# jannerm/ddpo

Measured on AMD Instinct MI355X. Metric: sampled images/sec (512^2, 50 DDIM steps), higher is better.
Workload: dtype f32 (f16mx: f16 MFMA + MX-fp8 cross terms on the long-reduction conv/GEMM layers, bf16x3-split MFMA elsewhere); 1 GPU; BASELINE configs[1]: compressed-animals geometry, sd15 U-Net+VAE (random init), 512x512, 50 DDIM steps, CFG 5.0, eta 1.0, sample_batch_size 8/GPU, VAE decode included; parallelism=dp1, global_batch=8

## Files before the change

ddpo_amd/csrc/attention_bf16.hip:

```cpp
#include "common.h"
#include <cstdlib>


typedef __bf16 bf16x8 __attribute__((ext_vector_type(8)));
typedef _Float16 f16x8 __attribute__((ext_vector_type(8)));
typedef _Float16 f16x2 __attribute__((ext_vector_type(2)));
typedef float f32x16 __attribute__((ext_vector_type(16)));

typedef __bf16 bf16x2 __attribute__((ext_vector_type(2)));
__device__ __forceinline__ uint32_t cvt_pk_bf16_a(float lo, float hi) {
  const bf16x2 v = {(__bf16)lo, (__bf16)hi};
  return __builtin_bit_cast(uint32_t, v);
}
__device__ __forceinline__ uint32_t cvt_pk_f16_a(float lo, float hi) {
  const f16x2 v = {(_Float16)lo, (_Float16)hi};
  return __builtin_bit_cast(uint32_t, v);
}
__device__ __forceinline__ void split2(float a, float b, uint32_t& hi, uint32_t& lo) {
  hi = cvt_pk_bf16_a(a, b);
  lo = cvt_pk_bf16_a(a - __uint_as_float(hi << 16), b - __uint_as_float(hi & 0xFFFF0000u));
}
__device__ __forceinline__ void split2h(float a, float b, uint32_t& hi, uint32_t& lo) {
  const float lim = 65504.f;
  a = fminf(fmaxf(a, -lim), lim);
// ... 87 lines not shown
                                                     bool& grew) {
  float mx = sacc[0][0];
#pragma unroll
  for (int j = 0; j < 2; ++j)
#pragma unroll
    for (int r = 0; r < 16; ++r) mx = fmaxf(mx, sacc[j][r]);
  mx = fmaxf(mx, __shfl_xor(mx, 32, 64));
  const float m_new = fmaxf(m_run, mx);
  alpha = __builtin_amdgcn_exp2f(m_run - m_new);
  grew = m_new > m_run;
  m_run = m_new;
  float ls = 0.f;
#pragma unroll
  for (int j = 0; j < 2; ++j) {
#pragma unroll
    for (int half = 0; half < 2; ++half) {
      uint32_t hi[4], lo[4];
#pragma unroll
      for (int e = 0; e < 4; ++e) {
        const float p0 = __builtin_amdgcn_exp2f(sacc[j][8 * half + 2 * e] - m_new);
        const float p1 = __builtin_amdgcn_exp2f(sacc[j][8 * half + 2 * e + 1] - m_new);
        ls += p0 + p1;
        split2(p0, p1, hi[e], lo[e]);
      }
      ph[2 * j + half] = __builtin_bit_cast(bf16x8, make_uint4(hi[0], hi[1], hi[2], hi[3]));
      pl[2 * j + half] = __builtin_bit_cast(bf16x8, make_uint4(lo[0], lo[1], lo[2], lo[3]));
    }
  }
  l_run = l_run * alpha + ls;
}

template <int NDT, int LDVT, int QB = 1>
__device__ __forceinline__ void attn_pv_tile_x3(const char* Vhi, const char* Vlo, int li, int h, const bf16x8 (*ph)[4], const bf16x8 (*pl)[4],
                                                f32x16 (*oacc)[NDT]) {
#pragma unroll
  for (int u = 0; u < 4; ++u) {
#pragma unroll
    for (int n = 0; n < NDT; ++n) {
      const int off = ((32 * n + li) * LDVT + 16 * u + 4 * h) * 2;
      const uint2 a0 = *reinterpret_cast<const uint2*>(Vhi + off), a1 = *reinterpret_cast<const uint2*>(Vhi + off + 16);
      const uint2 c0 = *reinterpret_cast<const uint2*>(Vlo + off), c1 = *reinterpret_cast<const uint2*>(Vlo + off + 16);
      const bf16x8 vh = __builtin_bit_cast(bf16x8, make_uint4(a0.x, a0.y, a1.x, a1.y));
      const bf16x8 vl = __builtin_bit_cast(bf16x8, make_uint4(c0.x, c0.y, c1.x, c1.y));
#pragma unroll
      for (int qb = 0; qb < QB; ++qb) {
        oacc[qb][n] = MFMA32(vl, ph[qb][u], oacc[qb][n]);
        oacc[qb][n] = MFMA32(vh, pl[qb][u], oacc[qb][n]);
        oacc[qb][n] = MFMA32(vh, ph[qb][u], oacc[qb][n]);
      }
    }
  }
}

template <bool F16P, bool ONES, int NDT, int LDVT>
__device__ __forceinline__ void attn_tile_tail(const f32x16 (&sacc)[2], float& m_run, float& l_run, f32x16 (&oacc)[NDT], const char* Vhi, const char* Vlo,
                                               int li, int h) {
  float alpha;
  bool grew;
  if constexpr (F16P) {
    f16x8 ph[4];
    attn_softmax_tile<ONES>(sacc, m_run, l_run, ph, alpha, grew);
    if (__any(grew)) {
#pragma unroll
      for (int n = 0; n < NDT; ++n)
#pragma unroll
        for (int r = 0; r < 16; ++r) oacc[n][r] *= alpha;
    }
    attn_pv_tile<NDT, LDVT>(Vhi, Vlo, li, h, &ph, &oacc);
  } else {
    bf16x8 ph[4], pl[4];
    attn_softmax_tile_x3(sacc, m_run, l_run, ph, pl, alpha, grew);
    if (__any(grew)) {
#pragma unroll
      for (int n = 0; n < NDT; ++n)
#pragma unroll
        for (int r = 0; r < 16; ++r) oacc[n][r] *= alpha;
    }
    attn_pv_tile_x3<NDT, LDVT>(Vhi, Vlo, li, h, &ph, &pl, &oacc);
  }
}

struct AttnOut {
  float* o;
  uint16_t* hi;
  uint16_t* lo;
  int ld;
  int64_t rows;
};
template <int D, int NDT>
__device__ __forceinline__ void attn_store_o(const AttnOut out, int64_t row, int col0, const f32x16 (&oacc)[NDT], float inv, int h) {
#pragma unroll
  for (int n = 0; n < NDT; ++n) {
#pragma unroll
    for (int g = 0; g < 4; ++g) {
      const int dc = 32 * n + 8 * g + 4 * h;
      if (dc >= D) continue;
      const float v0 = oacc[n][4 * g] * inv, v1 = oacc[n][4 * g + 1] * inv, v2 = oacc[n][4 * g + 2] * inv, v3 = oacc[n][4 * g + 3] * inv;
      if (out.hi) {
        uint32_t h0, l0, h1, l1;
        split2(v0, v1, h0, l0);
        split2(v2, v3, h1, l1);
        const int64_t off = plane_off(row, col0 + dc, out.ld, out.rows);
        *reinterpret_cast<uint2*>(out.hi + off) = make_uint2(h0, h1);
        *reinterpret_cast<uint2*>(out.lo + off) = make_uint2(l0, l1);
      } else {
        *reinterpret_cast<float4*>(out.o + row * out.ld + col0 + dc) = make_float4(v0, v1, v2, v3);
      }
    }
  }
}


template <int D, int DKP, int DVP, bool F16P>
__global__ void __launch_bounds__(256) attn_fwd_bf16_kernel(const float* __restrict__ q, int ldq, const float* __restrict__ k, int ldk,
                                                            const float* __restrict__ v, int ldv, const AttnOut out,
                                                            float* __restrict__ lse, int heads, int Nq, int Nk, float scale_log2e) {
  constexpr int KT = 64;
  constexpr int LDK = DKP + 8;
  constexpr int LDVT = KT + 4;
  constexpr int NKS = DKP / 16;
  constexpr int NDT = DVP / 32;
  constexpr bool ONES = F16P && DVP > D;
  constexpr int K_BYTES = KT * LDK * 2, VT_BYTES = DVP * LDVT * 2;
  __shared__ __attribute__((aligned(16))) char smem[2 * K_BYTES + 2 * VT_BYTES];
  char* Khi = smem; char* Klo = smem + K_BYTES;
  char* Vhi = smem + 2 * K_BYTES; char* Vlo = Vhi + VT_BYTES;

  const int t = threadIdx.x, lane = t & 63, wid = t >> 6;
  const int li = lane & 31, h = lane >> 5;
  const int bh = blockIdx.y, b = bh / heads, hd = bh - b * heads;
  const int q0 = blockIdx.x * 128 + wid * 32;
  const int qrow = min(q0 + li, Nq - 1);

  bf16x8 qh[NKS], ql[NKS];
  {
    const float* qp = q + ((int64_t)b * Nq + qrow) * ldq + hd * D;
#pragma unroll
    for (int s = 0; s < NKS; ++s) {
      uint32_t hi[4], lo[4];
#pragma unroll
      for (int e = 0; e < 4; ++e) {
        const int dk = 16 * s + 8 * h + 2 * e;
        const float a = dk < D ? qp[dk] * scale_log2e : 0.f;
        const float c = dk + 1 < D ? qp[dk + 1] * scale_log2e : 0.f;
        split2(a, c, hi[e], lo[e]);
      }
      qh[s] = __builtin_bit_cast(bf16x8, make_uint4(hi[0], hi[1], hi[2], hi[3]));
      ql[s] = __builtin_bit_cast(bf16x8, make_uint4(lo[0], lo[1], lo[2], lo[3]));
    }
  }
  for (int i = t; i < (2 * K_BYTES + 2 * VT_BYTES) / 16; i += 256) reinterpret_cast<uint4*>(smem)[i] = make_uint4(0u, 0u, 0u, 0u);
  if constexpr (ONES) {
    __syncthreads();
    if (t < KT) reinterpret_cast<uint16_t*>(Vhi)[D * LDVT + t] = (uint16_t)ATTN_F16_ONE;
  }

  f32x16 oacc[NDT];
#pragma unroll
  for (int n = 0; n < NDT; ++n)
#pragma unroll
    for (int r = 0; r < 16; ++r) oacc[n][r] = 0.f;
  float m_run = -INFINITY, l_run = 0.f;
  const float* kb = k + (int64_t)b * Nk * ldk + hd * D;
  const float* vb = v + (int64_t)b * Nk * ldv + hd * D;

  for (int kt0 = 0; kt0 < Nk; kt0 += KT) {
    __syncthreads();
    for (int i = t; i < KT * (D / 4); i += 256) {
      const int key = i / (D / 4), c4 = i - key * (D / 4);
      float4 kv = make_float4(0.f, 0.f, 0.f, 0.f), vv = kv;
      if (kt0 + key < Nk) {
        kv = *reinterpret_cast<const float4*>(kb + (int64_t)(kt0 + key) * ldk + c4 * 4);
        vv = *reinterpret_cast<const float4*>(vb + (int64_t)(kt0 + key) * ldv + c4 * 4);
      }
      uint32_t h0, l0, h1, l1;
      split2(kv.x, kv.y, h0, l0);
      split2(kv.z, kv.w, h1, l1);
      *reinterpret_cast<uint2*>(Khi + (key * LDK + c4 * 4) * 2) = make_uint2(h0, h1);
      *reinterpret_cast<uint2*>(Klo + (key * LDK + c4 * 4) * 2) = make_uint2(l0, l1);
      if (F16P) { split2h(vv.x, vv.y, h0, l0); split2h(vv.z, vv.w, h1, l1); }
      else { split2(vv.x, vv.y, h0, l0); split2(vv.z, vv.w, h1, l1); }
      uint16_t* vh = reinterpret_cast<uint16_t*>(Vhi);
      uint16_t* vl = reinterpret_cast<uint16_t*>(Vlo);
      const int d0 = c4 * 4;
      vh[(d0 + 0) * LDVT + key] = (uint16_t)(h0 & 0xFFFFu); vh[(d0 + 1) * LDVT + key] = (uint16_t)(h0 >> 16);
      vh[(d0 + 2) * LDVT + key] = (uint16_t)(h1 & 0xFFFFu); vh[(d0 + 3) * LDVT + key] = (uint16_t)(h1 >> 16);
      vl[(d0 + 0) * LDVT + key] = (uint16_t)(l0 & 0xFFFFu); vl[(d0 + 1) * LDVT + key] = (uint16_t)(l0 >> 16);
      vl[(d0 + 2) * LDVT + key] = (uint16_t)(l1 & 0xFFFFu); vl[(d0 + 3) * LDVT + key] = (uint16_t)(l1 >> 16);
    }
    __syncthreads();

    f32x16 sacc[2];
#pragma unroll
    for (int j = 0; j < 2; ++j)
#pragma unroll
      for (int r = 0; r < 16; ++r) sacc[j][r] = 0.f;
#pragma unroll
    for (int s = 0; s < NKS; ++s) {
#pragma unroll
      for (int j = 0; j < 2; ++j) {
        const int off = ((j * 32 + li) * LDK + 16 * s + 8 * h) * 2;
        const bf16x8 kh = *reinterpret_cast<const bf16x8*>(Khi + off);
        const bf16x8 kl = *reinterpret_cast<const bf16x8*>(Klo + off);
        sacc[j] = MFMA32(kl, qh[s], sacc[j]);
        sacc[j] = MFMA32(kh, ql[s], sacc[j]);
        sacc[j] = MFMA32(kh, qh[s], sacc[j]);
      }
    }
    if (kt0 + KT > Nk) {
#pragma unroll
      for (int j = 0; j < 2; ++j)
#pragma unroll
        for (int r = 0; r < 16; ++r)
          if (kt0 + 32 * j + (r & 3) + 8 * (r >> 2) + 4 * h >= Nk) sacc[j][r] = -INFINITY;
    }
    attn_tile_tail<F16P, ONES, NDT, LDVT>(sacc, m_run, l_run, oacc, Vhi, Vlo, li, h);
  }

  const float l_tot = attn_row_sum<D, NDT, ONES>(oacc, l_run, li);
  const float inv = 1.0f / l_tot;
  if (lse && h == 0 && q0 + li < Nq) lse[(int64_t)bh * Nq + q0 + li] = m_run + log2f(l_tot) - (F16P ? ATTN_P_SHIFT : 0.f);
  if (q0 + li < Nq) attn_store_o<D, NDT>(out, (int64_t)b * Nq + q0 + li, hd * D, oacc, inv, h);
}

template <int D, int DKP, int DVP>
struct AttnImg {
  static constexpr int KT = 64, LDK = DKP + 8, LDVT = KT + 4;
  static constexpr int K_BYTES = KT * LDK * 2, VT_BYTES = DVP * LDVT * 2;
  static constexpr int BYTES = 2 * K_BYTES + 2 * VT_BYTES;
  static constexpr int CHUNKS = BYTES / 16;
};

template <int D, int DKP, int DVP, bool F16P>
__global__ void __launch_bounds__(256) attn_pack_kv_kernel(const float* __restrict__ k, int ldk, const float* __restrict__ v, int ldv,
                                                           uint4* __restrict__ img, int heads, int Nk, int ntiles) {
  using I = AttnImg<D, DKP, DVP>;
  __shared__ __attribute__((aligned(16))) char smem[I::BYTES];
  char* Khi = smem; char* Klo = smem + I::K_BYTES;
  char* Vhi = smem + 2 * I::K_BYTES; char* Vlo = Vhi + I::VT_BYTES;
  const int t = threadIdx.x;
  const int tile = blockIdx.x, bh = blockIdx.y, b = bh / heads, hd = bh - b * heads;
  const int kt0 = tile * I::KT;
  for (int i = t; i < I::CHUNKS; i += 256) reinterpret_cast<uint4*>(smem)[i] = make_uint4(0u, 0u, 0u, 0u);
  __syncthreads();
  if (F16P && DVP > D && t < I::KT) reinterpret_cast<uint16_t*>(Vhi)[D * I::LDVT + t] = (uint16_t)ATTN_F16_ONE;
  const float* kb = k + (int64_t)b * Nk * ldk + hd * D;
  const float* vb = v + (int64_t)b * Nk * ldv + hd * D;
  for (int i = t; i < I::KT * (D / 4); i += 256) {
    const int key = i / (D / 4), c4 = i - key * (D / 4);
    if (kt0 + key >= Nk) continue;
    const float4 kv = *reinterpret_cast<const float4*>(kb + (int64_t)(kt0 + key) * ldk + c4 * 4);
    const float4 vv = *reinterpret_cast<const float4*>(vb + (int64_t)(kt0 + key) * ldv + c4 * 4);
    uint32_t h0, l0, h1, l1;
    split2(kv.x, kv.y, h0, l0);
    split2(kv.z, kv.w, h1, l1);
    *reinterpret_cast<uint2*>(Khi + (key * I::LDK + c4 * 4) * 2) = make_uint2(h0, h1);
    *reinterpret_cast<uint2*>(Klo + (key * I::LDK + c4 * 4) * 2) = make_uint2(l0, l1);
    if (F16P) { split2h(vv.x, vv.y, h0, l0); split2h(vv.z, vv.w, h1, l1); }
    else { split2(vv.x, vv.y, h0, l0); split2(vv.z, vv.w, h1, l1); }
    uint16_t* vh = reinterpret_cast<uint16_t*>(Vhi);
    uint16_t* vl = reinterpret_cast<uint16_t*>(Vlo);
    const int d0 = c4 * 4;
    vh[(d0 + 0) * I::LDVT + key] = (uint16_t)(h0 & 0xFFFFu); vh[(d0 + 1) * I::LDVT + key] = (uint16_t)(h0 >> 16);
    vh[(d0 + 2) * I::LDVT + key] = (uint16_t)(h1 & 0xFFFFu); vh[(d0 + 3) * I::LDVT + key] = (uint16_t)(h1 >> 16);
    vl[(d0 + 0) * I::LDVT + key] = (uint16_t)(l0 & 0xFFFFu); vl[(d0 + 1) * I::LDVT + key] = (uint16_t)(l0 >> 16);
    vl[(d0 + 2) * I::LDVT + key] = (uint16_t)(l1 & 0xFFFFu); vl[(d0 + 3) * I::LDVT + key] = (uint16_t)(l1 >> 16);
  }
  __syncthreads();
  uint4* dst = img + ((int64_t)bh * ntiles + tile) * I::CHUNKS;
  for (int i = t; i < I::CHUNKS; i += 256) dst[i] = reinterpret_cast<const uint4*>(smem)[i];
}

template <int D, int DKP, int DVP, bool F16P>
__global__ void __launch_bounds__(256, (DVP <= 32 ? 4 : (DKP <= 48 ? 3 : 2))) attn_fwd_bf16_pk_kernel(const float* __restrict__ q, int ldq, const uint4* __restrict__ img,
                                                               const AttnOut out, float* __restrict__ lse, int heads,
                                                               int Nq, int Nk, int ntiles, float scale_log2e) {
  using I = AttnImg<D, DKP, DVP>;
  constexpr int KT = I::KT, LDK = I::LDK, LDVT = I::LDVT;
  constexpr int NKS = DKP / 16, NDT = DVP / 32;
  constexpr bool ONES = F16P && DVP > D;
  constexpr int NCH = (I::CHUNKS + 255) / 256;
  __shared__ __attribute__((aligned(16))) char smem[I::BYTES];
  const char* Khi = smem; const char* Klo = smem + I::K_BYTES;
  const char* Vhi = smem + 2 * I::K_BYTES; const char* Vlo = Vhi + I::VT_BYTES;

  const int t = threadIdx.x, lane = t & 63, wid = t >> 6;
  const int li = lane & 31, h = lane >> 5;
  const int bh = blockIdx.y, b = bh / heads, hd = bh - b * heads;
  const int q0 = blockIdx.x * 128 + wid * 32;
  const int qrow = min(q0 + li, Nq - 1);

  bf16x8 qh[NKS], ql[NKS];
  {
    const float* qp = q + ((int64_t)b * Nq + qrow) * ldq + hd * D;
#pragma unroll
    for (int s = 0; s < NKS; ++s) {
      uint32_t hi[4], lo[4];
#pragma unroll
      for (int e = 0; e < 4; ++e) {
        const int dk = 16 * s + 8 * h + 2 * e;
        const float a = dk < D ? qp[dk] * scale_log2e : 0.f;
        const float c = dk + 1 < D ? qp[dk + 1] * scale_log2e : 0.f;
        split2(a, c, hi[e], lo[e]);
      }
      qh[s] = __builtin_bit_cast(bf16x8, make_uint4(hi[0], hi[1], hi[2], hi[3]));
      ql[s] = __builtin_bit_cast(bf16x8, make_uint4(lo[0], lo[1], lo[2], lo[3]));
    }
  }

  f32x16 oacc[NDT];
#pragma unroll
  for (int n = 0; n < NDT; ++n)
#pragma unroll
    for (int r = 0; r < 16; ++r) oacc[n][r] = 0.f;
  float m_run = -INFINITY, l_run = 0.f;

  const uint4* src = img + (int64_t)bh * ntiles * I::CHUNKS;
  uint4 pre[NCH];
#pragma unroll
  for (int c = 0; c < NCH; ++c) {
    const int i = t + 256 * c;
    pre[c] = (NCH * 256 == I::CHUNKS || i < I::CHUNKS) ? src[i] : make_uint4(0u, 0u, 0u, 0u);
  }

  for (int tile = 0; tile < ntiles; ++tile) {
    const int kt0 = tile * KT;
    __syncthreads();
#pragma unroll
    for (int c = 0; c < NCH; ++c) {
      const int i = t + 256 * c;
      if (NCH * 256 == I::CHUNKS || i < I::CHUNKS) reinterpret_cast<uint4*>(smem)[i] = pre[c];
    }
    __syncthreads();
    {
      const uint4* nsrc = src + (int64_t)min(tile + 1, ntiles - 1) * I::CHUNKS;
#pragma unroll
      for (int c = 0; c < NCH; ++c) {
        const int i = t + 256 * c;
        pre[c] = (NCH * 256 == I::CHUNKS || i < I::CHUNKS) ? nsrc[i] : make_uint4(0u, 0u, 0u, 0u);
      }
    }

    f32x16 sacc[2];
#pragma unroll
    for (int j = 0; j < 2; ++j)
#pragma unroll
      for (int r = 0; r < 16; ++r) sacc[j][r] = 0.f;
#pragma unroll
    for (int s = 0; s < NKS; ++s) {
#pragma unroll
      for (int j = 0; j < 2; ++j) {
        const int off = ((j * 32 + li) * LDK + 16 * s + 8 * h) * 2;
        const bf16x8 kh = *reinterpret_cast<const bf16x8*>(Khi + off);
        const bf16x8 kl = *reinterpret_cast<const bf16x8*>(Klo + off);
        sacc[j] = MFMA32(kl, qh[s], sacc[j]);
        sacc[j] = MFMA32(kh, ql[s], sacc[j]);
        sacc[j] = MFMA32(kh, qh[s], sacc[j]);
      }
    }
    if (kt0 + KT > Nk) {
#pragma unroll
      for (int j = 0; j < 2; ++j)
#pragma unroll
        for (int r = 0; r < 16; ++r)
          if (kt0 + 32 * j + (r & 3) + 8 * (r >> 2) + 4 * h >= Nk) sacc[j][r] = -INFINITY;
    }
    attn_tile_tail<F16P, ONES, NDT, LDVT>(sacc, m_run, l_run, oacc, Vhi, Vlo, li, h);
  }

  const float l_tot = attn_row_sum<D, NDT, ONES>(oacc, l_run, li);
  const float inv = 1.0f / l_tot;
  if (lse && h == 0 && q0 + li < Nq) lse[(int64_t)bh * Nq + q0 + li] = m_run + log2f(l_tot) - (F16P ? ATTN_P_SHIFT : 0.f);
  if (q0 + li < Nq) attn_store_o<D, NDT>(out, (int64_t)b * Nq + q0 + li, hd * D, oacc, inv, h);
}

typedef unsigned int u32x4_a __attribute__((ext_vector_type(4)));

template <int D, int DKP, int DVP, int QB, bool F16P>
__global__ void __launch_bounds__(256, (QB == 2 ? 2 : (DVP <= 32 ? 4 : (DKP <= 48 ? 3 : 2)))) attn_fwd_bf16_dma_kernel(const float* __restrict__ q, int ldq, const uint4* __restrict__ img,
                                                               const AttnOut out, float* __restrict__ lse, int heads,
                                                               int Nq, int Nk, int ntiles, float scale_log2e) {
  using I = AttnImg<D, DKP, DVP>;
  constexpr int KT = I::KT, LDK = I::LDK, LDVT = I::LDVT;
  constexpr int NKS = DKP / 16, NDT = DVP / 32;
  constexpr bool ONES = F16P && DVP > D;
  constexpr int KP = 2 * I::K_BYTES, VP = 2 * I::VT_BYTES;
  static_assert(KP % 1024 == 0 && VP % 1024 == 0, "LDS-DMA moves whole KiB pieces");
  constexpr int NPK = KP / 1024, NPV = VP / 1024;
  __shared__ __attribute__((aligned(1024))) char smem[2 * KP + VP];

  const int t = threadIdx.x, lane = t & 63, wid = t >> 6;
  const int wv = __builtin_amdgcn_readfirstlane(wid);
  const int li = lane & 31, h = lane >> 5;
  const int bh = blockIdx.y, b = bh / heads, hd = bh - b * heads;
  const int q0 = blockIdx.x * (128 * QB) + wid * (32 * QB);

  bf16x8 qh[QB][NKS], ql[QB][NKS];
#pragma unroll
  for (int qb = 0; qb < QB; ++qb) {
    const int qrow = min(q0 + 32 * qb + li, Nq - 1);
    const float* qp = q + ((int64_t)b * Nq + qrow) * ldq + hd * D;
#pragma unroll
    for (int s = 0; s < NKS; ++s) {
      uint32_t hi[4], lo[4];
#pragma unroll
      for (int e = 0; e < 4; ++e) {
        const int dk = 16 * s + 8 * h + 2 * e;
        const float a = dk < D ? qp[dk] * scale_log2e : 0.f;
        const float c = dk + 1 < D ? qp[dk + 1] * scale_log2e : 0.f;
        split2(a, c, hi[e], lo[e]);
      }
      qh[qb][s] = __builtin_bit_cast(bf16x8, make_uint4(hi[0], hi[1], hi[2], hi[3]));
      ql[qb][s] = __builtin_bit_cast(bf16x8, make_uint4(lo[0], lo[1], lo[2], lo[3]));
    }
  }

  f32x16 oacc[QB][NDT];
  float m_run[QB], l_run[QB];
#pragma unroll
  for (int qb = 0; qb < QB; ++qb) {
    m_run[qb] = -INFINITY; l_run[qb] = 0.f;
#pragma unroll
    for (int n = 0; n < NDT; ++n)
#pragma unroll
      for (int r = 0; r < 16; ++r) oacc[qb][n][r] = 0.f;
  }

  const uint64_t base = reinterpret_cast<uint64_t>(img + (int64_t)bh * ntiles * I::CHUNKS);
  const u32x4_a rs = {(uint32_t)base, (uint32_t)(base >> 32) & 0xFFFFu, 0x7FFFFFFFu, 0x00020000u};
  const uint32_t lds0 = (uint32_t)(uintptr_t)((__attribute__((address_space(3))) char*)smem);
  const uint32_t lane16 = (uint32_t)lane * 16u;
  auto fill = [&](uint32_t lds_region, uint32_t img_off, int npieces, int tile) {
    const uint32_t so = (uint32_t)tile * (uint32_t)I::BYTES + img_off;
    for (int p = wv; p < npieces; p += 4)
      asm volatile("s_nop 4\n\ts_mov_b32 m0, %0\n\ts_nop 0\n\tbuffer_load_dwordx4 %1, %2, %3 offen lds"
                   :: "s"(lds0 + lds_region + (uint32_t)p * 1024u), "v"(lane16 + (uint32_t)p * 1024u), "s"(rs), "s"(so) : "memory");
  };

  fill(0, 0, NPK, 0);
  for (int tile = 0; tile < ntiles; ++tile) {
    const int kt0 = tile * KT;
    const uint32_t kreg = (tile & 1) ? KP : 0;
    const char* Khi = smem + kreg; const char* Klo = Khi + I::K_BYTES;
    const char* Vhi = smem + 2 * KP; const char* Vlo = Vhi + I::VT_BYTES;
    asm volatile("s_waitcnt vmcnt(0) lgkmcnt(0)" ::: "memory");
    __builtin_amdgcn_s_barrier();
    fill(2 * KP, KP, NPV, tile);
    if (tile + 1 < ntiles) fill((tile & 1) ? 0 : KP, 0, NPK, tile + 1);

    f16x8 ph[QB][4];
    bf16x8 xh[QB][4], xl[QB][4];
#pragma unroll
    for (int qb = 0; qb < QB; ++qb) {
      f32x16 sacc[2];
  #pragma unroll
      for (int j = 0; j < 2; ++j)
  #pragma unroll
        for (int r = 0; r < 16; ++r) sacc[j][r] = 0.f;
  #pragma unroll
      for (int s = 0; s < NKS; ++s) {
  #pragma unroll
        for (int j = 0; j < 2; ++j) {
          const int off = ((j * 32 + li) * LDK + 16 * s + 8 * h) * 2;
          const bf16x8 kh = *reinterpret_cast<const bf16x8*>(Khi + off);
          const bf16x8 kl = *reinterpret_cast<const bf16x8*>(Klo + off);
          sacc[j] = MFMA32(kl, qh[qb][s], sacc[j]);
          sacc[j] = MFMA32(kh, ql[qb][s], sacc[j]);
          sacc[j] = MFMA32(kh, qh[qb][s], sacc[j]);
        }
      }
      if (kt0 + KT > Nk) {
  #pragma unroll
        for (int j = 0; j < 2; ++j)
  #pragma unroll
          for (int r = 0; r < 16; ++r)
            if (kt0 + 32 * j + (r & 3) + 8 * (r >> 2) + 4 * h >= Nk) sacc[j][r] = -INFINITY;
      }
      float alpha;
      bool grew;
      if constexpr (F16P) attn_softmax_tile<ONES>(sacc, m_run[qb], l_run[qb], ph[qb], alpha, grew);
      else attn_softmax_tile_x3(sacc, m_run[qb], l_run[qb], xh[qb], xl[qb], alpha, grew);
      if (__any(grew)) {
  #pragma unroll
        for (int n = 0; n < NDT; ++n)
  #pragma unroll
          for (int r = 0; r < 16; ++r) oacc[qb][n][r] *= alpha;
      }
    }
    asm volatile("s_waitcnt vmcnt(0) lgkmcnt(0)" ::: "memory");
    __builtin_amdgcn_s_barrier();
    if constexpr (F16P) attn_pv_tile<NDT, LDVT, QB>(Vhi, Vlo, li, h, ph, oacc);
    else attn_pv_tile_x3<NDT, LDVT, QB>(Vhi, Vlo, li, h, xh, xl, oacc);
  }

#pragma unroll
  for (int qb = 0; qb < QB; ++qb) {
    const int qi = q0 + 32 * qb + li;
    const float l_tot = attn_row_sum<D, NDT, ONES>(oacc[qb], l_run[qb], li);
    const float inv = 1.0f / l_tot;
    if (lse && h == 0 && qi < Nq) lse[(int64_t)bh * Nq + qi] = m_run[qb] + log2f(l_tot) - (F16P ? ATTN_P_SHIFT : 0.f);
    if (qi < Nq) attn_store_o<D, NDT>(out, (int64_t)b * Nq + qi, hd * D, oacc[qb], inv, h);
  }
}

#define ATTN_PK_MIN_NK 256

template <int D, int DKP, int DVP, bool F16P>
static int launch_pack_kv(const float* k, int ldk, const float* v, int ldv, uint4* img, int B, int heads, int Nk, hipStream_t st) {
  using I = AttnImg<D, DKP, DVP>;
  const int ntiles = (Nk + I::KT - 1) / I::KT;
  hipLaunchKernelGGL((attn_pack_kv_kernel<D, DKP, DVP, F16P>), dim3(ntiles, B * heads), dim3(256), 0, st, k, ldk, v, ldv, img, heads, Nk, ntiles);
  DDPO_LAUNCH_CHECK();
  return DDPO_OK;
}

template <int D, int DKP, int DVP, bool F16P>
static int launch_attn_images(const float* q, int ldq, const uint4* img, const AttnOut& out, float* lse, int B, int heads, int Nq, int Nk,
                              float scale, hipStream_t st) {
  using I = AttnImg<D, DKP, DVP>;
  dim3 grid((Nq + 127) / 128, B * heads);
  const int ntiles = (Nk + I::KT - 1) / I::KT;
  if constexpr ((2 * I::K_BYTES) % 1024 == 0 && (2 * I::VT_BYTES) % 1024 == 0) {
    if ((int64_t)ntiles * I::BYTES < 0x7FFFFFFF) {
      hipLaunchKernelGGL((attn_fwd_bf16_dma_kernel<D, DKP, DVP, 1, F16P>), grid, dim3(256), 0, st, q, ldq, img, out, lse, heads, Nq, Nk, ntiles,
                         scale * 1.4426950408889634f);
      DDPO_LAUNCH_CHECK();
      return DDPO_OK;
    }
  }
  hipLaunchKernelGGL((attn_fwd_bf16_pk_kernel<D, DKP, DVP, F16P>), grid, dim3(256), 0, st, q, ldq, img, out, lse, heads, Nq, Nk, ntiles,
                     scale * 1.4426950408889634f);
  DDPO_LAUNCH_CHECK();
  return DDPO_OK;
}

template <int D, int DKP, int DVP, bool F16P>
static int launch_attn_bf16(const float* q, int ldq, const float* k, int ldk, const float* v, int ldv, const AttnOut& out, float* lse,
                            int B, int heads, int Nq, int Nk, float scale, void* ws, size_t ws_bytes, hipStream_t st) {
  using I = AttnImg<D, DKP, DVP>;
  dim3 grid((Nq + 127) / 128, B * heads);
  const int ntiles = (Nk + I::KT - 1) / I::KT;
  const size_t need = (size_t)B * heads * ntiles * I::BYTES;
  if (Nk >= ATTN_PK_MIN_NK && ws && ws_bytes >= need && !(reinterpret_cast<uintptr_t>(ws) & 15)) {
    uint4* img = reinterpret_cast<uint4*>(ws);
    const int rc = launch_pack_kv<D, DKP, DVP, F16P>(k, ldk, v, ldv, img, B, heads, Nk, st);
    if (rc != DDPO_OK) return rc;
    return launch_attn_images<D, DKP, DVP, F16P>(q, ldq, img, out, lse, B, heads, Nq, Nk, scale, st);
  }
  hipLaunchKernelGGL((attn_fwd_bf16_kernel<D, DKP, DVP, F16P>), grid, dim3(256), 0, st, q, ldq, k, ldk, v, ldv, out, lse, heads, Nq, Nk,
                     scale * 1.4426950408889634f);
  DDPO_LAUNCH_CHECK();
  return DDPO_OK;
}

template <int D, int DKP, int DVP>
static size_t attn_img_bytes(int B, int heads, int Nk) {
  using I = AttnImg<D, DKP, DVP>;
  return (size_t)B * heads * ((Nk + I::KT - 1) / I::KT) * I::BYTES;
}
template <int D, int DKP, int DVP>
static size_t attn_ws(int B, int heads, int Nk) {
  if (Nk < ATTN_PK_MIN_NK) return 0;
  return attn_img_bytes<D, DKP, DVP>(B, heads, Nk);
}

extern "C" size_t ddpo_attention_fwd_bf16x3_ws_bytes(int B, int heads, int Nk, int d) {
  if (B <= 0 || heads <= 0 || Nk <= 0) return 0;
  switch (d) {
    case 8:  return attn_ws<8, 16, 32>(B, heads, Nk);
    case 16: return attn_ws<16, 16, 32>(B, heads, Nk);
    case 40: return attn_ws<40, 48, 64>(B, heads, Nk);
    case 64: return attn_ws<64, 64, 64>(B, heads, Nk);
    case 80: return attn_ws<80, 80, 96>(B, heads, Nk);
    default: return 0;
  }
}

#define ATTN_BY_D(CALL)                                      \
  switch (d) {                                               \
    case 8:  return CALL(8, 16, 32);                         \
    case 16: return CALL(16, 16, 32);                        \
    case 40: return CALL(40, 48, 64);                        \
    case 64: return CALL(64, 64, 64);                        \
    case 80: return CALL(80, 80, 96);                        \
    default: return DDPO_EINVAL;  \
  }

static bool attn_out_ok(const AttnOut& out, int heads, int d) {
  if (out.hi) {
    if (!out.lo || out.o || (out.ld & 3) || ((reinterpret_cast<uintptr_t>(out.hi) | reinterpret_cast<uintptr_t>(out.lo)) & 7)) return false;
    return out.ld != 0 || ((heads * d) & 31) == 0;
  }
  return out.o && !(out.ld & 3) && !(reinterpret_cast<uintptr_t>(out.o) & 15);
}

template <bool F16P>
static int attention_fwd_impl(const float* q, int ldq, const float* k, int ldk, const float* v, int ldv, const AttnOut& out,
                              float* lse, int B, int heads, int Nq, int Nk, int d, float scale, void* ws, size_t ws_bytes, void* stream) {
  if (!q || !k || !v || B <= 0 || heads <= 0 || Nq <= 0 || Nk <= 0 || d <= 0 || !attn_out_ok(out, heads, d)) return DDPO_EINVAL;
  if ((ldq & 3) || (ldk & 3) || (ldv & 3) || (long)B * heads > 65535) return DDPO_EINVAL;
  if ((reinterpret_cast<uintptr_t>(q) | reinterpret_cast<uintptr_t>(k) | reinterpret_cast<uintptr_t>(v)) & 15) return DDPO_EINVAL;
  hipStream_t st = as_stream(stream);
#define CALL(DD, DK, DV) launch_attn_bf16<DD, DK, DV, F16P>(q, ldq, k, ldk, v, ldv, out, lse, B, heads, Nq, Nk, scale, ws, ws_bytes, st)
  ATTN_BY_D(CALL)
#undef CALL
}
extern "C" int ddpo_attention_fwd_bf16x3(const float* q, int ldq, const float* k, int ldk, const float* v, int ldv, float* o, int ldo,
                                         float* lse, int B, int heads, int Nq, int Nk, int d, float scale, void* ws, size_t ws_bytes,
                                         void* stream) {
  return attention_fwd_impl<false>(q, ldq, k, ldk, v, ldv, AttnOut{o, nullptr, nullptr, ldo, (int64_t)B * Nq}, lse, B, heads, Nq, Nk, d, scale, ws,
// ... 94 lines not shown
```

Baseline: 4.204 images/sec.

## Pack hi/lo split into shared MFMA K-chunks for head dim 40 f16 attention

```diff
diff --git a/ddpo_amd/csrc/attention_bf16.hip b/ddpo_amd/csrc/attention_bf16.hip
--- a/ddpo_amd/csrc/attention_bf16.hip
+++ b/ddpo_amd/csrc/attention_bf16.hip
@@ -163,7 +163,133 @@
   }
 }
 
-template <bool F16P, bool ONES, int NDT, int LDVT>
+template <int D, int DKP, int DVP, bool F16P = false>
+struct AttnImg {
+  static constexpr bool RS = F16P && D == 40;
+  static constexpr int KT = 64;
+  static constexpr int LDK = RS ? 2 * D + 8 : DKP + 8;
+  static constexpr int LDVT = KT + 4;
+  static constexpr int VROWS = RS ? 96 : DVP;
+  static constexpr int K_BYTES = KT * LDK * 2, VT_BYTES = VROWS * LDVT * 2;
+  static constexpr int KP = RS ? K_BYTES : 2 * K_BYTES;
+  static constexpr int VP = RS ? (VT_BYTES + 1023) / 1024 * 1024 : 2 * VT_BYTES;
+  static constexpr int KLO = RS ? 2 * D : K_BYTES;
+  static constexpr int VLO = RS ? 0 : VT_BYTES;
+  static constexpr int NKS = DKP / 16;
+  static constexpr int NQF = RS ? 8 : 2 * NKS;
+  static constexpr int NACC = RS ? 3 : DVP / 32;
+  static constexpr int BYTES = KP + VP;
+  static constexpr int CHUNKS = BYTES / 16;
+  __device__ static int vlo_row(int d) { return RS ? (d < 32 ? 64 + d : 16 + d) : d; }
+};
+
+__device__ __forceinline__ int attn_rs_kchunk(int u, int h) {
+  return u < 5 ? (h ? u : 5 + u) : (u < 7 ? 2 * (u - 5) + h : (h ? 10 : 4));
+}
+template <class I, int D>
+__device__ __forceinline__ void attn_q_frags(const float* qp, float scale_log2e, int h, bf16x8* qf) {
+  if constexpr (I::RS) {
+    uint4 hi[5], lo[5];
+#pragma unroll
+    for (int c = 0; c < 5; ++c) {
+      uint32_t a[4], b[4];
+#pragma unroll
+      for (int e = 0; e < 4; ++e) split2(qp[8 * c + 2 * e] * scale_log2e, qp[8 * c + 2 * e + 1] * scale_log2e, a[e], b[e]);
+      hi[c] = make_uint4(a[0], a[1], a[2], a[3]);
+      lo[c] = make_uint4(b[0], b[1], b[2], b[3]);
+    }
+#pragma unroll
+    for (int u = 0; u < 5; ++u) qf[u] = __builtin_bit_cast(bf16x8, h ? lo[u] : hi[u]);
+    qf[5] = __builtin_bit_cast(bf16x8, h ? hi[1] : hi[0]);
+    qf[6] = __builtin_bit_cast(bf16x8, h ? hi[3] : hi[2]);
+    qf[7] = __builtin_bit_cast(bf16x8, h ? make_uint4(0u, 0u, 0u, 0u) : hi[4]);
+  } else {
+#pragma unroll
+    for (int s = 0; s < I::NKS; ++s) {
+      uint32_t hi[4], lo[4];
+#pragma unroll
+      for (int e = 0; e < 4; ++e) {
+        const int dk = 16 * s + 8 * h + 2 * e;
+        const float a = dk < D ? qp[dk] * scale_log2e : 0.f;
+        const float c = dk + 1 < D ? qp[dk + 1] * scale_log2e : 0.f;
+        split2(a, c, hi[e], lo[e]);
+      }
+      qf[2 * s] = __builtin_bit_cast(bf16x8, make_uint4(hi[0], hi[1], hi[2], hi[3]));
+      qf[2 * s + 1] = __builtin_bit_cast(bf16x8, make_uint4(lo[0], lo[1], lo[2], lo[3]));
+    }
+  }
+}
+
+template <class I>
+__device__ __forceinline__ void attn_scores(const char* K, int li, int h, const bf16x8* qf, f32x16 (&sacc)[2]) {
+#pragma unroll
+  for (int j = 0; j < 2; ++j)
+#pragma unroll
+    for (int r = 0; r < 16; ++r) sacc[j][r] = 0.f;
+  if constexpr (I::RS) {
+#pragma unroll
+    for (int u = 0; u < 8; ++u) {
+#pragma unroll
+      for (int j = 0; j < 2; ++j) {
+        const bf16x8 ka = *reinterpret_cast<const bf16x8*>(K + (j * 32 + li) * I::LDK * 2 + 16 * attn_rs_kchunk(u, h));
+        sacc[j] = MFMA32(ka, qf[u], sacc[j]);
+      }
+    }
+  } else {
+#pragma unroll
+    for (int s = 0; s < I::NKS; ++s) {
+#pragma unroll
+      for (int j = 0; j < 2; ++j) {
+        const int off = ((j * 32 + li) * I::LDK + 16 * s + 8 * h) * 2;
+        const bf16x8 kh = *reinterpret_cast<const bf16x8*>(K + off);
+        const bf16x8 kl = *reinterpret_cast<const bf16x8*>(K + I::K_BYTES + off);
+        sacc[j] = MFMA32(kl, qf[2 * s], sacc[j]);
+        sacc[j] = MFMA32(kh, qf[2 * s + 1], sacc[j]);
+        sacc[j] = MFMA32(kh, qf[2 * s], sacc[j]);
+      }
+    }
+  }
+}
+
+template <int LDVT, int QB = 1>
+__device__ __forceinline__ void attn_pv_tile_rs(const char* V, int li, int h, const f16x8 (*ph)[4], f32x16 (*oacc)[3]) {
+  f16x8 va[2][3];
+  auto fetch = [&](int u, int slot) {
+#pragma unroll
+    for (int n = 0; n < 3; ++n) {
+      const int off = ((32 * n + li) * LDVT + 16 * u + 4 * h) * 2;
+      const uint2 a0 = *reinterpret_cast<const uint2*>(V + off), a1 = *reinterpret_cast<const uint2*>(V + off + 16);
+      va[slot][n] = __builtin_bit_cast(f16x8, make_uint4(a0.x, a0.y, a1.x, a1.y));
+    }
+  };
+  fetch(0, 0);
+#pragma unroll
+  for (int u = 0; u < 4; ++u) {
+    if (u + 1 < 4) fetch(u + 1, (u + 1) & 1);
+    __builtin_amdgcn_sched_barrier(0);
+#pragma unroll
+    for (int qb = 0; qb < QB; ++qb)
+#pragma unroll
+      for (int n = 0; n < 3; ++n) oacc[qb][n] = MFMA32H(va[u & 1][n], ph[qb][u], oacc[qb][n]);
+    __builtin_amdgcn_sched_barrier(0);
+  }
+}
+
+template <bool RS, int NACC, int NDT>
+__device__ __forceinline__ void attn_unstack(const f32x16 (&a)[NACC], f32x16 (&o)[NDT]) {
+  if constexpr (RS) {
+    static_assert(NACC == 3 && NDT == 2, "RS: 3 accumulator tiles -> 2 output tiles");
+    o[0] = a[0] + a[2];
+    o[1] = a[1];
+#pragma unroll
+    for (int i = 0; i < 4; ++i) o[1][i] = a[1][i] + a[1][8 + i];
+  } else {
+#pragma unroll
+    for (int n = 0; n < NDT; ++n) o[n] = a[n];
+  }
+}
+
+template <bool F16P, bool ONES, int NDT, int LDVT, bool RS = false>
 __device__ __forceinline__ void attn_tile_tail(const f32x16 (&sacc)[2], float& m_run, float& l_run, f32x16 (&oacc)[NDT], const char* Vhi, const char* Vlo,
                                                int li, int h) {
   float alpha;
@@ -177,7 +303,8 @@
 #pragma unroll
         for (int r = 0; r < 16; ++r) oacc[n][r] *= alpha;
     }
-    attn_pv_tile<NDT, LDVT>(Vhi, Vlo, li, h, &ph, &oacc);
+    if constexpr (RS) attn_pv_tile_rs<LDVT>(Vhi, li, h, &ph, &oacc);
+    else attn_pv_tile<NDT, LDVT>(Vhi, Vlo, li, h, &ph, &oacc);
   } else {
     bf16x8 ph[4], pl[4];
     attn_softmax_tile_x3(sacc, m_run, l_run, ph, pl, alpha, grew);
@@ -223,19 +350,17 @@
 
 
 template <int D, int DKP, int DVP, bool F16P>
-__global__ void __launch_bounds__(256) attn_fwd_bf16_kernel(const float* __restrict__ q, int ldq, const float* __restrict__ k, int ldk,
+__global__ void __launch_bounds__(256, (AttnImg<D, DKP, DVP, F16P>::RS ? 3 : 1)) attn_fwd_bf16_kernel(const float* __restrict__ q, int ldq, const float* __restrict__ k, int ldk,
                                                             const float* __restrict__ v, int ldv, const AttnOut out,
                                                             float* __restrict__ lse, int heads, int Nq, int Nk, float scale_log2e) {
-  constexpr int KT = 64;
-  constexpr int LDK = DKP + 8;
-  constexpr int LDVT = KT + 4;
-  constexpr int NKS = DKP / 16;
+  using I = AttnImg<D, DKP, DVP, F16P>;
+  constexpr int KT = I::KT, LDK = I::LDK, LDVT = I::LDVT;
   constexpr int NDT = DVP / 32;
+  constexpr int NACC = I::NACC;
   constexpr bool ONES = F16P && DVP > D;
-  constexpr int K_BYTES = KT * LDK * 2, VT_BYTES = DVP * LDVT * 2;
-  __shared__ __attribute__((aligned(16))) char smem[2 * K_BYTES + 2 * VT_BYTES];
-  char* Khi = smem; char* Klo = smem + K_BYTES;
-  char* Vhi = smem + 2 * K_BYTES; char* Vlo = Vhi + VT_BYTES;
+  __shared__ __attribute__((aligned(16))) char smem[I::BYTES];
+  char* Khi = smem; char* Klo = smem + I::KLO;
+  char* Vhi = smem + I::KP; char* Vlo = Vhi + I::VLO;
 
   const int t = threadIdx.x, lane = t & 63, wid = t >> 6;
   const int li = lane & 31, h = lane >> 5;
@@ -243,32 +368,17 @@
   const int q0 = blockIdx.x * 128 + wid * 32;
   const int qrow = min(q0 + li, Nq - 1);
 
-  bf16x8 qh[NKS], ql[NKS];
-  {
-    const float* qp = q + ((int64_t)b * Nq + qrow) * ldq + hd * D;
-#pragma unroll
-    for (int s = 0; s < NKS; ++s) {
-      uint32_t hi[4], lo[4];
-#pragma unroll
-      for (int e = 0; e < 4; ++e) {
-        const int dk = 16 * s + 8 * h + 2 * e;
-        const float a = dk < D ? qp[dk] * scale_log2e : 0.f;
-        const float c = dk + 1 < D ? qp[dk + 1] * scale_log2e : 0.f;
-        split2(a, c, hi[e], lo[e]);
-      }
-      qh[s] = __builtin_bit_cast(bf16x8, make_uint4(hi[0], hi[1], hi[2], hi[3]));
-      ql[s] = __builtin_bit_cast(bf16x8, make_uint4(lo[0], lo[1], lo[2], lo[3]));
-    }
-  }
-  for (int i = t; i < (2 * K_BYTES + 2 * VT_BYTES) / 16; i += 256) reinterpret_cast<uint4*>(smem)[i] = make_uint4(0u, 0u, 0u, 0u);
+  bf16x8 qf[I::NQF];
+  attn_q_frags<I, D>(q + ((int64_t)b * Nq + qrow) * ldq + hd * D, scale_log2e, h, qf);
+  for (int i = t; i < I::BYTES / 16; i += 256) reinterpret_cast<uint4*>(smem)[i] = make_uint4(0u, 0u, 0u, 0u);
   if constexpr (ONES) {
     __syncthreads();
     if (t < KT) reinterpret_cast<uint16_t*>(Vhi)[D * LDVT + t] = (uint16_t)ATTN_F16_ONE;
   }
 
-  f32x16 oacc[NDT];
-#pragma unroll
-  for (int n = 0; n < NDT; ++n)
+  f32x16 oacc[NACC];
+#pragma unroll
+  for (int n = 0; n < NACC; ++n)
 #pragma unroll
     for (int r = 0; r < 16; ++r) oacc[n][r] = 0.f;
   float m_run = -INFINITY, l_run = 0.f;
@@ -293,31 +403,16 @@
       else { split2(vv.x, vv.y, h0, l0); split2(vv.z, vv.w, h1, l1); }
       uint16_t* vh = reinterpret_cast<uint16_t*>(Vhi);
       uint16_t* vl = reinterpret_cast<uint16_t*>(Vlo);
-      const int d0 = c4 * 4;
+      const int d0 = c4 * 4, dl = I::vlo_row(d0);
       vh[(d0 + 0) * LDVT + key] = (uint16_t)(h0 & 0xFFFFu); vh[(d0 + 1) * LDVT + key] = (uint16_t)(h0 >> 16);
       vh[(d0 + 2) * LDVT + key] = (uint16_t)(h1 & 0xFFFFu); vh[(d0 + 3) * LDVT + key] = (uint16_t)(h1 >> 16);
-      vl[(d0 + 0) * LDVT + key] = (uint16_t)(l0 & 0xFFFFu); vl[(d0 + 1) * LDVT + key] = (uint16_t)(l0 >> 16);
-      vl[(d0 + 2) * LDVT + key] = (uint16_t)(l1 & 0xFFFFu); vl[(d0 + 3) * LDVT + key] = (uint16_t)(l1 >> 16);
+      vl[(dl + 0) * LDVT + key] = (uint16_t)(l0 & 0xFFFFu); vl[(dl + 1) * LDVT + key] = (uint16_t)(l0 >> 16);
+      vl[(dl + 2) * LDVT + key] = (uint16_t)(l1 & 0xFFFFu); vl[(dl + 3) * LDVT + key] = (uint16_t)(l1 >> 16);
     }
     __syncthreads();
 
     f32x16 sacc[2];
-#pragma unroll
-    for (int j = 0; j < 2; ++j)
-#pragma unroll
-      for (int r = 0; r < 16; ++r) sacc[j][r] = 0.f;
-#pragma unroll
-    for (int s = 0; s < NKS; ++s) {
-#pragma unroll
-      for (int j = 0; j < 2; ++j) {
-        const int off = ((j * 32 + li) * LDK + 16 * s + 8 * h) * 2;
-        const bf16x8 kh = *reinterpret_cast<const bf16x8*>(Khi + off);
-        const bf16x8 kl = *reinterpret_cast<const bf16x8*>(Klo + off);
-        sacc[j] = MFMA32(kl, qh[s], sacc[j]);
-        sacc[j] = MFMA32(kh, ql[s], sacc[j]);
-        sacc[j] = MFMA32(kh, qh[s], sacc[j]);
-      }
-    }
+    attn_scores<I>(Khi, li, h, qf, sacc);
     if (kt0 + KT > Nk) {
 #pragma unroll
       for (int j = 0; j < 2; ++j)
@@ -325,30 +420,24 @@
         for (int r = 0; r < 16; ++r)
           if (kt0 + 32 * j + (r & 3) + 8 * (r >> 2) + 4 * h >= Nk) sacc[j][r] = -INFINITY;
     }
-    attn_tile_tail<F16P, ONES, NDT, LDVT>(sacc, m_run, l_run, oacc, Vhi, Vlo, li, h);
-  }
-
-  const float l_tot = attn_row_sum<D, NDT, ONES>(oacc, l_run, li);
+    attn_tile_tail<F16P, ONES, NACC, LDVT, I::RS>(sacc, m_run, l_run, oacc, Vhi, Vlo, li, h);
+  }
+
+  f32x16 o[NDT];
+  attn_unstack<I::RS>(oacc, o);
+  const float l_tot = attn_row_sum<D, NDT, ONES>(o, l_run, li);
   const float inv = 1.0f / l_tot;
   if (lse && h == 0 && q0 + li < Nq) lse[(int64_t)bh * Nq + q0 + li] = m_run + log2f(l_tot) - (F16P ? ATTN_P_SHIFT : 0.f);
-  if (q0 + li < Nq) attn_store_o<D, NDT>(out, (int64_t)b * Nq + q0 + li, hd * D, oacc, inv, h);
-}
-
-template <int D, int DKP, int DVP>
-struct AttnImg {
-  static constexpr int KT = 64, LDK = DKP + 8, LDVT = KT + 4;
-  static constexpr int K_BYTES = KT * LDK * 2, VT_BYTES = DVP * LDVT * 2;
-  static constexpr int BYTES = 2 * K_BYTES + 2 * VT_BYTES;
-  static constexpr int CHUNKS = BYTES / 16;
-};
+  if (q0 + li < Nq) attn_store_o<D, NDT>(out, (int64_t)b * Nq + q0 + li, hd * D, o, inv, h);
+}
 
 template <int D, int DKP, int DVP, bool F16P>
 __global__ void __launch_bounds__(256) attn_pack_kv_kernel(const float* __restrict__ k, int ldk, const float* __restrict__ v, int ldv,
                                                            uint4* __restrict__ img, int heads, int Nk, int ntiles) {
-  using I = AttnImg<D, DKP, DVP>;
+  using I = AttnImg<D, DKP, DVP, F16P>;
   __shared__ __attribute__((aligned(16))) char smem[I::BYTES];
-  char* Khi = smem; char* Klo = smem + I::K_BYTES;
-  char* Vhi = smem + 2 * I::K_BYTES; char* Vlo = Vhi + I::VT_BYTES;
+  char* Khi = smem; char* Klo = smem + I::KLO;
+  char* Vhi = smem + I::KP; char* Vlo = Vhi + I::VLO;
   const int t = threadIdx.x;
   const int tile = blockIdx.x, bh = blockIdx.y, b = bh / heads, hd = bh - b * heads;
   const int kt0 = tile * I::KT;
@@ -371,11 +460,11 @@
     else { split2(vv.x, vv.y, h0, l0); split2(vv.z, vv.w, h1, l1); }
     uint16_t* vh = reinterpret_cast<uint16_t*>(Vhi);
     uint16_t* vl = reinterpret_cast<uint16_t*>(Vlo);
-    const int d0 = c4 * 4;
+    const int d0 = c4 * 4, dl = I::vlo_row(d0);
     vh[(d0 + 0) * I::LDVT + key] = (uint16_t)(h0 & 0xFFFFu); vh[(d0 + 1) * I::LDVT + key] = (uint16_t)(h0 >> 16);
     vh[(d0 + 2) * I::LDVT + key] = (uint16_t)(h1 & 0xFFFFu); vh[(d0 + 3) * I::LDVT + key] = (uint16_t)(h1 >> 16);
-    vl[(d0 + 0) * I::LDVT + key] = (uint16_t)(l0 & 0xFFFFu); vl[(d0 + 1) * I::LDVT + key] = (uint16_t)(l0 >> 16);
-    vl[(d0 + 2) * I::LDVT + key] = (uint16_t)(l1 & 0xFFFFu); vl[(d0 + 3) * I::LDVT + key] = (uint16_t)(l1 >> 16);
+    vl[(dl + 0) * I::LDVT + key] = (uint16_t)(l0 & 0xFFFFu); vl[(dl + 1) * I::LDVT + key] = (uint16_t)(l0 >> 16);
+    vl[(dl + 2) * I::LDVT + key] = (uint16_t)(l1 & 0xFFFFu); vl[(dl + 3) * I::LDVT + key] = (uint16_t)(l1 >> 16);
   }
   __syncthreads();
   uint4* dst = img + ((int64_t)bh * ntiles + tile) * I::CHUNKS;
@@ -386,14 +475,14 @@
 __global__ void __launch_bounds__(256, (DVP <= 32 ? 4 : (DKP <= 48 ? 3 : 2))) attn_fwd_bf16_pk_kernel(const float* __restrict__ q, int ldq, const uint4* __restrict__ img,
                                                                const AttnOut out, float* __restrict__ lse, int heads,
                                                                int Nq, int Nk, int ntiles, float scale_log2e) {
-  using I = AttnImg<D, DKP, DVP>;
-  constexpr int KT = I::KT, LDK = I::LDK, LDVT = I::LDVT;
-  constexpr int NKS = DKP / 16, NDT = DVP / 32;
+  using I = AttnImg<D, DKP, DVP, F16P>;
+  constexpr int KT = I::KT, LDVT = I::LDVT;
+  constexpr int NDT = DVP / 32, NACC = I::NACC;
   constexpr bool ONES = F16P && DVP > D;
   constexpr int NCH = (I::CHUNKS + 255) / 256;
   __shared__ __attribute__((aligned(16))) char smem[I::BYTES];
-  const char* Khi = smem; const char* Klo = smem + I::K_BYTES;
-  const char* Vhi = smem + 2 * I::K_BYTES; const char* Vlo = Vhi + I::VT_BYTES;
+  const char* Khi = smem;
+  const char* Vhi = smem + I::KP; const char* Vlo = Vhi + I::VLO;
 
   const int t = threadIdx.x, lane = t & 63, wid = t >> 6;
   const int li = lane & 31, h = lane >> 5;
@@ -401,27 +490,12 @@
   const int q0 = blockIdx.x * 128 + wid * 32;
   const int qrow = min(q0 + li, Nq - 1);
 
-  bf16x8 qh[NKS], ql[NKS];
-  {
-    const float* qp = q + ((int64_t)b * Nq + qrow) * ldq + hd * D;
-#pragma unroll
-    for (int s = 0; s < NKS; ++s) {
-      uint32_t hi[4], lo[4];
-#pragma unroll
-      for (int e = 0; e < 4; ++e) {
-        const int dk = 16 * s + 8 * h + 2 * e;
-        const float a = dk < D ? qp[dk] * scale_log2e : 0.f;
-        const float c = dk + 1 < D ? qp[dk + 1] * scale_log2e : 0.f;
-        split2(a, c, hi[e], lo[e]);
-      }
-      qh[s] = __builtin_bit_cast(bf16x8, make_uint4(hi[0], hi[1], hi[2], hi[3]));
-      ql[s] = __builtin_bit_cast(bf16x8, make_uint4(lo[0], lo[1], lo[2], lo[3]));
-    }
-  }
-
-  f32x16 oacc[NDT];
-#pragma unroll
-  for (int n = 0; n < NDT; ++n)
+  bf16x8 qf[I::NQF];
+  attn_q_frags<I, D>(q + ((int64_t)b * Nq + qrow) * ldq + hd * D, scale_log2e, h, qf);
+
+  f32x16 oacc[NACC];
+#pragma unroll
+  for (int n = 0; n < NACC; ++n)
 #pragma unroll
     for (int r = 0; r < 16; ++r) oacc[n][r] = 0.f;
   float m_run = -INFINITY, l_run = 0.f;
@@ -453,22 +527,7 @@
     }
 
     f32x16 sacc[2];
-#pragma unroll
-    for (int j = 0; j < 2; ++j)
-#pragma unroll
-      for (int r = 0; r < 16; ++r) sacc[j][r] = 0.f;
-#pragma unroll
-    for (int s = 0; s < NKS; ++s) {
-#pragma unroll
-      for (int j = 0; j < 2; ++j) {
-        const int off = ((j * 32 + li) * LDK + 16 * s + 8 * h) * 2;
-        const bf16x8 kh = *reinterpret_cast<const bf16x8*>(Khi + off);
-        const bf16x8 kl = *reinterpret_cast<const bf16x8*>(Klo + off);
-        sacc[j] = MFMA32(kl, qh[s], sacc[j]);
-        sacc[j] = MFMA32(kh, ql[s], sacc[j]);
-        sacc[j] = MFMA32(kh, qh[s], sacc[j]);
-      }
-    }
+    attn_scores<I>(Khi, li, h, qf, sacc);
     if (kt0 + KT > Nk) {
 #pragma unroll
       for (int j = 0; j < 2; ++j)
@@ -476,13 +535,15 @@
         for (int r = 0; r < 16; ++r)
           if (kt0 + 32 * j + (r & 3) + 8 * (r >> 2) + 4 * h >= Nk) sacc[j][r] = -INFINITY;
     }
-    attn_tile_tail<F16P, ONES, NDT, LDVT>(sacc, m_run, l_run, oacc, Vhi, Vlo, li, h);
-  }
-
-  const float l_tot = attn_row_sum<D, NDT, ONES>(oacc, l_run, li);
+    attn_tile_tail<F16P, ONES, NACC, LDVT, I::RS>(sacc, m_run, l_run, oacc, Vhi, Vlo, li, h);
+  }
+
+  f32x16 o[NDT];
+  attn_unstack<I::RS>(oacc, o);
+  const float l_tot = attn_row_sum<D, NDT, ONES>(o, l_run, li);
   const float inv = 1.0f / l_tot;
   if (lse && h == 0 && q0 + li < Nq) lse[(int64_t)bh * Nq + q0 + li] = m_run + log2f(l_tot) - (F16P ? ATTN_P_SHIFT : 0.f);
-  if (q0 + li < Nq) attn_store_o<D, NDT>(out, (int64_t)b * Nq + q0 + li, hd * D, oacc, inv, h);
+  if (q0 + li < Nq) attn_store_o<D, NDT>(out, (int64_t)b * Nq + q0 + li, hd * D, o, inv, h);
 }
 
 typedef unsigned int u32x4_a __attribute__((ext_vector_type(4)));
@@ -491,11 +552,11 @@
 __global__ void __launch_bounds__(256, (QB == 2 ? 2 : (DVP <= 32 ? 4 : (DKP <= 48 ? 3 : 2)))) attn_fwd_bf16_dma_kernel(const float* __restrict__ q, int ldq, const uint4* __restrict__ img,
                                                                const AttnOut out, float* __restrict__ lse, int heads,
                                                                int Nq, int Nk, int ntiles, float scale_log2e) {
-  using I = AttnImg<D, DKP, DVP>;
-  constexpr int KT = I::KT, LDK = I::LDK, LDVT = I::LDVT;
-  constexpr int NKS = DKP / 16, NDT = DVP / 32;
+  using I = AttnImg<D, DKP, DVP, F16P>;
+  constexpr int KT = I::KT, LDVT = I::LDVT;
+  constexpr int NDT = DVP / 32, NACC = I::NACC;
   constexpr bool ONES = F16P && DVP > D;
-  constexpr int KP = 2 * I::K_BYTES, VP = 2 * I::VT_BYTES;
+  constexpr int KP = I::KP, VP = I::VP;
   static_assert(KP % 1024 == 0 && VP % 1024 == 0, "LDS-DMA moves whole KiB pieces");
   constexpr int NPK = KP / 1024, NPV = VP / 1024;
   __shared__ __attribute__((aligned(1024))) char smem[2 * KP + VP];
@@ -506,33 +567,20 @@
   const int bh = blockIdx.y, b = bh / heads, hd = bh - b * heads;
   const int q0 = blockIdx.x * (128 * QB) + wid * (32 * QB);
 
-  bf16x8 qh[QB][NKS], ql[QB][NKS];
+  bf16x8 qf[QB][I::NQF];
 #pragma unroll
   for (int qb = 0; qb < QB; ++qb) {
     const int qrow = min(q0 + 32 * qb + li, Nq - 1);
-    const float* qp = q + ((int64_t)b * Nq + qrow) * ldq + hd * D;
-#pragma unroll
-    for (int s = 0; s < NKS; ++s) {
-      uint32_t hi[4], lo[4];
-#pragma unroll
-      for (int e = 0; e < 4; ++e) {
-        const int dk = 16 * s + 8 * h + 2 * e;
-        const float a = dk < D ? qp[dk] * scale_log2e : 0.f;
-        const float c = dk + 1 < D ? qp[dk + 1] * scale_log2e : 0.f;
-        split2(a, c, hi[e], lo[e]);
-      }
-      qh[qb][s] = __builtin_bit_cast(bf16x8, make_uint4(hi[0], hi[1], hi[2], hi[3]));
-      ql[qb][s] = __builtin_bit_cast(bf16x8, make_uint4(lo[0], lo[1], lo[2], lo[3]));
-    }
-  }
-
-  f32x16 oacc[QB][NDT];
+    attn_q_frags<I, D>(q + ((int64_t)b * Nq + qrow) * ldq + hd * D, scale_log2e, h, qf[qb]);
+  }
+
+  f32x16 oacc[QB][NACC];
   float m_run[QB], l_run[QB];
 #pragma unroll
   for (int qb = 0; qb < QB; ++qb) {
     m_run[qb] = -INFINITY; l_run[qb] = 0.f;
 #pragma unroll
-    for (int n = 0; n < NDT; ++n)
+    for (int n = 0; n < NACC; ++n)
 #pragma unroll
       for (int r = 0; r < 16; ++r) oacc[qb][n][r] = 0.f;
   }
@@ -552,8 +600,8 @@
   for (int tile = 0; tile < ntiles; ++tile) {
     const int kt0 = tile * KT;
     const uint32_t kreg = (tile & 1) ? KP : 0;
-    const char* Khi = smem + kreg; const char* Klo = Khi + I::K_BYTES;
-    const char* Vhi = smem + 2 * KP; const char* Vlo = Vhi + I::VT_BYTES;
+    const char* Khi = smem + kreg;
+    const char* Vhi = smem + 2 * KP; const char* Vlo = Vhi + I::VLO;
     asm volatile("s_waitcnt vmcnt(0) lgkmcnt(0)" ::: "memory");
     __builtin_amdgcn_s_barrier();
     fill(2 * KP, KP, NPV, tile);
@@ -564,22 +612,7 @@
 #pragma unroll
     for (int qb = 0; qb < QB; ++qb) {
       f32x16 sacc[2];
-  #pragma unroll
-      for (int j = 0; j < 2; ++j)
-  #pragma unroll
-        for (int r = 0; r < 16; ++r) sacc[j][r] = 0.f;
-  #pragma unroll
-      for (int s = 0; s < NKS; ++s) {
-  #pragma unroll
-        for (int j = 0; j < 2; ++j) {
-          const int off = ((j * 32 + li) * LDK + 16 * s + 8 * h) * 2;
-          const bf16x8 kh = *reinterpret_cast<const bf16x8*>(Khi + off);
-          const bf16x8 kl = *reinterpret_cast<const bf16x8*>(Klo + off);
-          sacc[j] = MFMA32(kl, qh[qb][s], sacc[j]);
-          sacc[j] = MFMA32(kh, ql[qb][s], sacc[j]);
-          sacc[j] = MFMA32(kh, qh[qb][s], sacc[j]);
-        }
-      }
+      attn_scores<I>(Khi, li, h, qf[qb], sacc);
       if (kt0 + KT > Nk) {
   #pragma unroll
         for (int j = 0; j < 2; ++j)
@@ -593,24 +626,27 @@
       else attn_softmax_tile_x3(sacc, m_run[qb], l_run[qb], xh[qb], xl[qb], alpha, grew);
       if (__any(grew)) {
   #pragma unroll
-        for (int n = 0; n < NDT; ++n)
+        for (int n = 0; n < NACC; ++n)
   #pragma unroll
           for (int r = 0; r < 16; ++r) oacc[qb][n][r] *= alpha;
       }
     }
     asm volatile("s_waitcnt vmcnt(0) lgkmcnt(0)" ::: "memory");
     __builtin_amdgcn_s_barrier();
-    if constexpr (F16P) attn_pv_tile<NDT, LDVT, QB>(Vhi, Vlo, li, h, ph, oacc);
+    if constexpr (I::RS) attn_pv_tile_rs<LDVT, QB>(Vhi, li, h, ph, oacc);
+    else if constexpr (F16P) attn_pv_tile<NDT, LDVT, QB>(Vhi, Vlo, li, h, ph, oacc);
     else attn_pv_tile_x3<NDT, LDVT, QB>(Vhi, Vlo, li, h, xh, xl, oacc);
   }
 
 #pragma unroll
   for (int qb = 0; qb < QB; ++qb) {
     const int qi = q0 + 32 * qb + li;
-    const float l_tot = attn_row_sum<D, NDT, ONES>(oacc[qb], l_run[qb], li);
+    f32x16 o[NDT];
+    attn_unstack<I::RS>(oacc[qb], o);
+    const float l_tot = attn_row_sum<D, NDT, ONES>(o, l_run[qb], li);
     const float inv = 1.0f / l_tot;
     if (lse && h == 0 && qi < Nq) lse[(int64_t)bh * Nq + qi] = m_run[qb] + log2f(l_tot) - (F16P ? ATTN_P_SHIFT : 0.f);
-    if (qi < Nq) attn_store_o<D, NDT>(out, (int64_t)b * Nq + qi, hd * D, oacc[qb], inv, h);
+    if (qi < Nq) attn_store_o<D, NDT>(out, (int64_t)b * Nq + qi, hd * D, o, inv, h);
   }
 }
 
@@ -618,7 +654,7 @@
 
 template <int D, int DKP, int DVP, bool F16P>
 static int launch_pack_kv(const float* k, int ldk, const float* v, int ldv, uint4* img, int B, int heads, int Nk, hipStream_t st) {
-  using I = AttnImg<D, DKP, DVP>;
+  using I = AttnImg<D, DKP, DVP, F16P>;
   const int ntiles = (Nk + I::KT - 1) / I::KT;
   hipLaunchKernelGGL((attn_pack_kv_kernel<D, DKP, DVP, F16P>), dim3(ntiles, B * heads), dim3(256), 0, st, k, ldk, v, ldv, img, heads, Nk, ntiles);
   DDPO_LAUNCH_CHECK();
@@ -628,10 +664,10 @@
 template <int D, int DKP, int DVP, bool F16P>
 static int launch_attn_images(const float* q, int ldq, const uint4* img, const AttnOut& out, float* lse, int B, int heads, int Nq, int Nk,
                               float scale, hipStream_t st) {
-  using I = AttnImg<D, DKP, DVP>;
+  using I = AttnImg<D, DKP, DVP, F16P>;
   dim3 grid((Nq + 127) / 128, B * heads);
   const int ntiles = (Nk + I::KT - 1) / I::KT;
-  if constexpr ((2 * I::K_BYTES) % 1024 == 0 && (2 * I::VT_BYTES) % 1024 == 0) {
+  if constexpr (I::KP % 1024 == 0 && I::VP % 1024 == 0) {
     if ((int64_t)ntiles * I::BYTES < 0x7FFFFFFF) {
       hipLaunchKernelGGL((attn_fwd_bf16_dma_kernel<D, DKP, DVP, 1, F16P>), grid, dim3(256), 0, st, q, ldq, img, out, lse, heads, Nq, Nk, ntiles,
                          scale * 1.4426950408889634f);
@@ -648,7 +684,7 @@
 template <int D, int DKP, int DVP, bool F16P>
 static int launch_attn_bf16(const float* q, int ldq, const float* k, int ldk, const float* v, int ldv, const AttnOut& out, float* lse,
                             int B, int heads, int Nq, int Nk, float scale, void* ws, size_t ws_bytes, hipStream_t st) {
-  using I = AttnImg<D, DKP, DVP>;
+  using I = AttnImg<D, DKP, DVP, F16P>;
   dim3 grid((Nq + 127) / 128, B * heads);
   const int ntiles = (Nk + I::KT - 1) / I::KT;
   const size_t need = (size_t)B * heads * ntiles * I::BYTES;
@@ -667,6 +703,7 @@
 template <int D, int DKP, int DVP>
 static size_t attn_img_bytes(int B, int heads, int Nk) {
   using I = AttnImg<D, DKP, DVP>;
+  static_assert(AttnImg<D, DKP, DVP, true>::BYTES <= I::BYTES, "the f16p image must fit the shared size");
   return (size_t)B * heads * ((Nk + I::KT - 1) / I::KT) * I::BYTES;
 }
 template <int D, int DKP, int DVP>
```

After: 4.261 images/sec, median of 6. 1.01x the previous value.
